# KleistLab/ADAPTed

Hardware: AMD Instinct MI355X
Metric: reads/sec (adapter+polyA detect), RNA004 200k-sample reads (higher is better)
Workload: dtype f32 samples/statistics, f64 cumulative sums + LLR trace

## Files before the change

### adapted_amd/csrc/adapted_hip.hip

```cpp
#include <hip/hip_runtime.h>

#include <cmath>
#include <cstdio>
#include <cstring>
#include <cstdlib>
#include <string>
#include <vector>

#include "adapted_hip.h"
#include "handle.h"
#include "common.h"
__device__ unsigned long long g_dbg[ADP_NDBG] = {0};
__device__ unsigned long long g_bs_tally[ADP_NTALLY][8] = {{0}};
#include "llr_stream.h"
#include "n1_select.h"
#include "n1_fused.h"
#include "peaks.h"
#include "synth.h"
#include "validate.h"
#include "cand_stats2.h"
#include "series_pipe.h"
#include "cnn_topk.h"
#include "cnn_conv.h"
#include "cnn_conv_split.h"
// ... 445 lines not shown
    hipStream_t st = h->stream;
    MbState *mbs = h->mbs.as<MbState>();
    uint32_t *gh = h->ghist.as<uint32_t>(), *gb = h->gbelow.as<uint32_t>();
    unsigned long long *gc = h->gcnt.as<unsigned long long>();
    const int collect = ((long long)minibatch * T >= (1ll << 24)) ? 1 : 0;
    ALLOCCHK(collect && h->cbuf.ensure((size_t)n_mb * N1_CB_CAP * 4));
    uint32_t *cb = h->cbuf.as<uint32_t>();
    int bpm = 4096 / n_mb; if (bpm > 256) bpm = 256; if (bpm < 4) bpm = 4;
    dim3 hg(bpm, n_mb), pg(n_mb);
    const int pdiv = 32;
    int col_div = 1;
    if (T >= 8192) { col_div = T / (pdiv * 96); if (col_div > 64) col_div = 64; if (col_div < 2) col_div = 2; }
    int row_step = (col_div > 1) ? 1 : minibatch / 32; if (row_step < 1) row_step = 1;
    int sb = (minibatch + row_step - 1) / row_step; if (sb > bpm) sb = bpm; if (sb < 1) sb = 1;
    dim3 sg(sb, n_mb);
    const double thr = h->cfg.sig_norm_outlier_thresh;
    const long long fused_min = getenv("ADP_N1_FUSED_MIN") ? atoll(getenv("ADP_N1_FUSED_MIN")) : (1ll << 22);
    if ((long long)minibatch * T >= fused_min && T >= 64) {
        ALLOCCHK(h->cbuf.ensure((size_t)n_mb * N1_CB_CAP * 4) || h->fz.ensure((size_t)n_mb * sizeof(N1Fused)) ||
                 h->fcnt.ensure((size_t)n_mb * 8 * N1F_NCNT) || h->n1heavy.ensure((size_t)n_mb * N1H_WORDS * 4));
        cb = h->cbuf.as<uint32_t>();
        N1Fused *fz = h->fz.as<N1Fused>();
        unsigned long long *fc = h->fcnt.as<unsigned long long>();
        HIPCHK(hipMemsetAsync(fc, 0, (size_t)n_mb * 8 * N1F_NCNT, st));
        uint32_t *hvy = h->n1heavy.as<uint32_t>();
        HIPCHK(hipMemsetAsync(hvy, 0, (size_t)n_mb * N1H_WORDS * 4, st));
        { Scope s(h, !profile ? nullptr : "k_n1 sample passes");
        const int s0 = (col_div > 1 && minibatch >= 64) ? env_int("ADP_N1_S0", 8) : 1;
        for (int mode = 0; mode < 2; mode++) {
            hipLaunchKernelGGL((k_n1_hist<0, SIG>), sg, dim3(N1_THREADS), 0, st, dsig, n, m, T, minibatch, mode, mbs, gh, gb, gc, row_step * (s0 > 1 ? s0 : 1), N1_ALWAYS, cb, 0, col_div, pdiv, tails);
            hipLaunchKernelGGL((k_n1_pick<0, N1_SAMPLE>), pg, dim3(256), 0, st, mbs, gh, gb, gc, mode, thr);
            hipLaunchKernelGGL((k_n1_hist<1, SIG>), sg, dim3(N1_THREADS), 0, st, dsig, n, m, T, minibatch, mode, mbs, gh, gb, gc, row_step, N1_ALWAYS, cb, 0, col_div, pdiv, tails);
            hipLaunchKernelGGL((k_n1_pick<1, N1_SAMPLE>), pg, dim3(256), 0, st, mbs, gh, gb, gc, mode, thr);
            hipLaunchKernelGGL(k_n1_fuse_setup, dim3((n_mb + 63) / 64), dim3(64), 0, st, mbs, fz, n_mb, mode);
        }
        hipLaunchKernelGGL(k_n1_heavy_scan<SIG>, dim3((sb + 3) / 4, n_mb), dim3(N1_THREADS), 0, st, dsig, n, m, T, minibatch, mbs, fz, hvy, row_step * 4, col_div, pdiv, tails);
        hipLaunchKernelGGL(k_n1_heavy_pick, pg, dim3(64), 0, st, mbs, fz, hvy, n_mb); }
        { Scope s(h, !profile ? nullptr : "k_n1_fused");
          hipLaunchKernelGGL(k_n1_fused<SIG>, hg, dim3(N1_THREADS), 0, st, dsig, n, m, T, minibatch, mbs, fz, fc, (float *)cb, hvy, tails); }
        { Scope s(h, !profile ? nullptr : "k_n1_fused_finish");
          hipLaunchKernelGGL(k_n1_fused_finish, pg, dim3(1024), 0, st, mbs, fz, fc, (const float *)cb, thr, (const uint32_t *)hvy); }
    }
    if ((long long)minibatch * T >= fused_min && T >= 64 && bpm < 128) hg = dim3(128, n_mb);
    for (int mode = 0; mode < 2; mode++) {
        hipLaunchKernelGGL((k_n1_hist<0, SIG>), sg, dim3(N1_THREADS), 0, st, dsig, n, m, T, minibatch, mode, mbs, gh, gb, gc, row_step, N1_ALWAYS, cb, 0, col_div, pdiv, tails);
        hipLaunchKernelGGL((k_n1_pick<0, N1_SAMPLE>), pg, dim3(256), 0, st, mbs, gh, gb, gc, mode, thr);
        hipLaunchKernelGGL((k_n1_hist<1, SIG>), sg, dim3(N1_THREADS), 0, st, dsig, n, m, T, minibatch, mode, mbs, gh, gb, gc, row_step, N1_ALWAYS, cb, 0, col_div, pdiv, tails);
        hipLaunchKernelGGL((k_n1_pick<1, N1_SAMPLE>), pg, dim3(256), 0, st, mbs, gh, gb, gc, mode, thr);
        { Scope s(h, !profile ? nullptr : (mode ? "k_n1_hist<1> mad" : "k_n1_hist<1> med"));
          hipLaunchKernelGGL((k_n1_hist<1, SIG>), hg, dim3(N1_THREADS), 0, st, dsig, n, m, T, minibatch, mode, mbs, gh, gb, gc, 1, N1_ALWAYS, cb, collect, 1, 8, tails); }
        hipLaunchKernelGGL((k_n1_pick<1, N1_FULL>), pg, dim3(256), 0, st, mbs, gh, gb, gc, mode, thr);
        hipLaunchKernelGGL(k_n1_finish, pg, dim3(1024), 0, st, mbs, cb, gc, gb, mode, thr);
        hipLaunchKernelGGL((k_n1_hist<0, SIG>), hg, dim3(N1_THREADS), 0, st, dsig, n, m, T, minibatch, mode, mbs, gh, gb, gc, 1, N1_IF_BAD, cb, 0, 1, 8, tails);
        hipLaunchKernelGGL((k_n1_pick<0, N1_FALLBACK>), pg, dim3(256), 0, st, mbs, gh, gb, gc, mode, thr);
        hipLaunchKernelGGL((k_n1_hist<1, SIG>), hg, dim3(N1_THREADS), 0, st, dsig, n, m, T, minibatch, mode, mbs, gh, gb, gc, 1, N1_IF_BAD, cb, 0, 1, 8, tails);
        hipLaunchKernelGGL((k_n1_pick<1, N1_FALLBACK>), pg, dim3(256), 0, st, mbs, gh, gb, gc, mode, thr);
        { Scope s(h, !profile ? nullptr : (mode ? "k_n1_hist<2> mad" : "k_n1_hist<2> med"));
          hipLaunchKernelGGL((k_n1_hist<2, SIG>), hg, dim3(N1_THREADS), 0, st, dsig, n, m, T, minibatch, mode, mbs, gh, gb, gc, 1, N1_IF_NOT_DONE, cb, 0, 1, 8, tails); }
        hipLaunchKernelGGL((k_n1_pick<2, N1_FULL>), pg, dim3(256), 0, st, mbs, gh, gb, gc, mode, thr);
    }
    return 0;
}

struct PhaseSync {
    hipEvent_t wait[3] = {nullptr, nullptr, nullptr};
    hipEvent_t done[3] = {nullptr, nullptr, nullptr};
};

static __device__ __host__ inline SigF32 sig_from(const SigF32 &s, size_t r0, int m) { return SigF32{s.base + r0 * (size_t)m}; }
static __device__ __host__ inline SigI16 sig_from(const SigI16 &s, size_t r0, int m) { return SigI16{s.base + r0 * (size_t)m, s.scale + r0, s.offset + r0, s.full_len + r0}; }
static inline SigIdx sig_subset(const SigF32 &s, const int32_t *sel) { return SigIdx{s.base, sel}; }
static inline SigIdxI16 sig_subset(const SigI16 &s, const int32_t *sel) { return SigIdxI16{s.base, s.scale, s.offset, s.full_len, sel}; }

static void launch_cumsum(adp_handle *h, int n)
{
    const int split = env_int("ADP_CUMSUM_GATHER", 1) != 0;
    hipLaunchKernelGGL(k_cumsum, dim3((n + 63) / 64), dim3(64), 0, h->stream, h->down.as<float>(), h->nvalid.as<int32_t>(), h->Lp, n,
                       h->nck, h->ck.as<double2>(), h->tail.as<double2>(), split);
    if (split)
        hipLaunchKernelGGL(k_cumsum_gather, dim3((n + 63) / 64), dim3(64), 0, h->stream, h->down.as<float>(), h->nvalid.as<int32_t>(), h->Lp, n,
                           h->nck, h->ck.as<double2>(), h->tail.as<double2>());
}

static void launch_polya_peak(adp_handle *h, int n, int mbsize, const double *pkv)
{
    const int grid = n < h->pslots ? n : h->pslots;
    hipLaunchKernelGGL(k_polya_peak, dim3(grid), dim3(64), (size_t)(((h->Lp / 2 + 1) + 8) / 16 + 2) * 4, h->stream, h->trace.as<double>(), h->nvalid.as<int32_t>(), h->Lp,
                       h->bmax.as<double>(), h->bmin.as<double>(), h->nsum, h->adapter_idx.as<int32_t>(), n, mbsize, h->mbs.as<MbState>(),
                       h->pk.as<int32_t>(), h->mk.as<uint32_t>(), h->polya_idx.as<int32_t>(), h->npk.as<int32_t>(), pkv, env_int("ADP_PK_PREFIX", PK_PREFIX));
}

template <class SIG>
static int llr_enqueue(adp_handle *h, SIG dsig, const int32_t *dlen, int n, int m, int minibatch, int flags,
                       adp_row *rows_dev, int rows_kind , int32_t *mb_status_dev, double *mb_params_dev,
                       int upto, const PhaseSync *ps)
{
    int rc = 0;
    const int n_mb = (n + minibatch - 1) / minibatch;
    h->last_n = n; h->last_nmb = n_mb;
    ALLOCCHK(h->mbs.ensure((size_t)n_mb * sizeof(MbState)) || h->ghist.ensure((size_t)n_mb * N1_BINS * 4) || h->gbelow.ensure((size_t)n_mb * 8) || h->gcnt.ensure((size_t)n_mb * 8 * N1_NCNT));
    rc = alloc_all(h, n, true);
    if (rc) return rc;
    hipStream_t st = h->stream;
#ifdef ADP_ABLATE
    sync_ablate(h);
#endif
    if (ps && ps->wait[0]) HIPCHK(hipStreamWaitEvent(st, ps->wait[0], 0));
    MbState *mbs = h->mbs.as<MbState>();
    HIPCHK(hipMemsetAsync(mbs, 0, (size_t)n_mb * sizeof(MbState), st));
    HIPCHK(hipMemsetAsync(h->ghist.p, 0, (size_t)n_mb * N1_BINS * 4, st));
    HIPCHK(hipMemsetAsync(h->gbelow.p, 0, (size_t)n_mb * 8, st));
    HIPCHK(hipMemsetAsync(h->gcnt.p, 0, (size_t)n_mb * 8 * N1_NCNT, st));
    const int T = h->T;
    bool sp_forked = false, sp_done = false;
    if (h->L <= 0) {
        hipLaunchKernelGGL(k_mb_set_status, dim3((n_mb + 255) / 256), dim3(256), 0, st, mbs, n_mb, ADP_MB_EMPTY_TRACE);
        if (ps) for (int k = 0; k < 2; k++) { if (k && ps->wait[k]) HIPCHK(hipStreamWaitEvent(st, ps->wait[k], 0)); if (ps->done[k]) HIPCHK(hipEventRecord(ps->done[k], st)); }
    } else {
        const int32_t *tails = (flags & ADP_TAILS_NAN) ? dlen : nullptr;
        rc = launch_n1(h, dsig, n, m, T, minibatch, n_mb, true, tails);
        if (rc) return rc;
        const bool sp_fused = upto >= 8 && (flags & ADP_WITH_START_PEAK) && h->layout == ADP_LAYOUT_MINIBATCH &&
                              h->cfg.sp_downscale_factor == h->ds && h->off % h->ds == 0 && T > h->off && env_int("ADP_SP_FUSED", 1) != 0;
        if (sp_fused) {
            ALLOCCHK(h->sphead.ensure((size_t)n * sizeof(SpHead)));
            Scope s(h, "k_sp_head");
            hipLaunchKernelGGL(k_sp_head<SIG>, dim3(n), dim3(64), (size_t)64 * h->cfg.sp_downscale_factor * 4, st, dsig, dlen, n, m, h->cfg, h->off, h->sphead.as<SpHead>());
        }
        if (upto >= 2 && sp_fused) {
            { Scope s(h, "k_norm_pool");
              auto kern = (h->ds == 10 && std::is_same<SIG, SigF32>::value && env_int("ADP_NP_PREFETCH", 1)) ? k_norm_pool<SIG, true, 5> : k_norm_pool<SIG, true, 0>;
              hipLaunchKernelGGL(kern, dim3(n), dim3(256), (size_t)NP_TILE * h->ds * 4, st, dsig, m, T, h->off, h->ds, h->L, h->Lp,
                                 minibatch, mbs, h->down.as<float>(), h->nvalid.as<int32_t>(), (const int64_t *)nullptr,
                                 dlen, (flags & ADP_TAILS_NAN) ? 1 : 0, h->sphead.as<SpHead>(), (float)h->cfg.open_pore_pa); }
            const int cov0 = h->off / h->ds, cov1 = cov0 + (T - h->off) / h->ds;
            Scope s(h, "k_sp_tail");
            hipLaunchKernelGGL(k_sp_tail<SIG>, dim3(n), dim3(64), (size_t)64 * h->cfg.sp_downscale_factor * 4, st, dsig, dlen, n, m, h->cfg, cov0, cov1,
                               (const SpHead *)h->sphead.as<SpHead>(), h->sp.as<SpOut>());
            sp_done = true;
        } else if (upto >= 2) {
            Scope s(h, "k_norm_pool");
            const int64_t *rng = nullptr;
            if (h->layout == ADP_LAYOUT_SINGLE_READ) {
                ALLOCCHK(h->rng0.ensure((size_t)n * 16));
                std::vector<int64_t> hr((size_t)2 * n);
                for (int i = 0; i < n; i++) { hr[2 * i] = 0; hr[2 * i + 1] = T; }
                HIPCHK(hipMemcpyAsync(h->rng0.p, hr.data(), (size_t)n * 16, hipMemcpyHostToDevice, st));
                HIPCHK(hipStreamSynchronize(st));
                rng = h->rng0.as<int64_t>();
            }
            auto kern = (h->ds == 10 && !rng && std::is_same<SIG, SigF32>::value && env_int("ADP_NP_PREFETCH", 1)) ? k_norm_pool<SIG, false, 5> : k_norm_pool<SIG, false, 0>;
            hipLaunchKernelGGL(kern, dim3(n), dim3(256), (size_t)NP_TILE * h->ds * 4, st, dsig, m, T, h->off, h->ds, h->L, h->Lp,
                               minibatch, mbs, h->down.as<float>(), h->nvalid.as<int32_t>(), rng,
                               dlen, (flags & ADP_TAILS_NAN) ? 1 : 0, (SpHead *)nullptr, 0.f);
        }
        if (upto >= 2)
            hipLaunchKernelGGL(k_check_empty, dim3((n + 255) / 256), dim3(256), 0, st, h->nvalid.as<int32_t>(), n, minibatch, mbs);
        if (ps && ps->done[0]) HIPCHK(hipEventRecord(ps->done[0], st));
        if (upto >= 8 && (flags & ADP_WITH_START_PEAK) && !sp_fused) {
            HIPCHK(hipEventRecord(h->ev_fork, st));
            HIPCHK(hipStreamWaitEvent(h->stream2, h->ev_fork, 0));
            { Scope s(h, "k_start_peak", h->stream2);
              hipLaunchKernelGGL(k_start_peak<SIG>, dim3(n), dim3(64), (size_t)64 * h->cfg.sp_downscale_factor * 4, h->stream2, dsig, dlen, n, m, h->cfg, h->sp.as<SpOut>()); }
            HIPCHK(hipEventRecord(h->ev_join, h->stream2));
            sp_forked = true;
        }
        if (ps && ps->wait[1]) HIPCHK(hipStreamWaitEvent(st, ps->wait[1], 0));
        if (upto >= 3) {
            Scope s(h, "k_cumsum");
            launch_cumsum(h, n);
        }
        if (upto >= 4) {
            Scope s(h, "k_gains<1>");
            hipLaunchKernelGGL(k_gains<1>, dim3((n + GAINS_WPB - 1) / GAINS_WPB), dim3(64 * GAINS_WPB), 0, st, h->down.as<float>(), h->nvalid.as<int32_t>(), h->Lp, h->nck,
                               h->ck.as<double2>(), h->tail.as<double2>(), h->adapter_idx.as<int32_t>(), minibatch, mbs,
                               h->trace.as<double>(), h->bmax.as<double>(), h->bmin.as<double>(), h->nsum, h->t1.as<int2>(), 0, h->pk.as<int32_t>(), h->npk.as<int32_t>(), h->Lp / 2 + 1, h->gstat.as<double>(), n, h->oh1);
        }
        if (upto >= 5) {
            Scope s(h, "k_adapter_peak");
            hipLaunchKernelGGL(k_adapter_peak, dim3(n), dim3(64), 0, st, h->trace.as<double>(), h->nvalid.as<int32_t>(), h->Lp,
                               h->bmax.as<double>(), h->bmin.as<double>(), h->nsum, h->t1.as<int2>(), minibatch, mbs,
                               h->cfg.adapter_peak_prominence, h->cfg.adapter_peak_rel_height,
                               h->cfg.adapter_peak_width / h->ds, h->adapter_idx.as<int32_t>(), h->gstat.as<double>());
        }
        double *pkvp = (env_int("ADP_PK_VALUES", 1) && h->pkv.cap >= (size_t)n * (h->Lp / 2 + 1) * 8) ? h->pkv.as<double>() : nullptr;
        if (upto >= 6) {
            Scope s(h, "k_gains<2>");
            hipLaunchKernelGGL(k_gains<2>, dim3((n + GAINS_WPB - 1) / GAINS_WPB), dim3(64 * GAINS_WPB), 0, st, h->down.as<float>(), h->nvalid.as<int32_t>(), h->Lp, h->nck,
                               h->ck.as<double2>(), h->tail.as<double2>(), h->adapter_idx.as<int32_t>(), minibatch, mbs,
                               h->trace.as<double>(), h->bmax.as<double>(), h->bmin.as<double>(), h->nsum, h->t1.as<int2>(), 0, h->pk.as<int32_t>(), h->npk.as<int32_t>(), h->Lp / 2 + 1, h->gstat.as<double>(), n, 5, pkvp);
        }
        if (upto >= 7) {
            Scope s(h, "k_polya_peak");
            launch_polya_peak(h, n, minibatch, pkvp);
        }
        if (ps && ps->done[1]) HIPCHK(hipEventRecord(ps->done[1], st));
    }
    if (upto >= 8) {
        if (ps && ps->wait[2]) HIPCHK(hipStreamWaitEvent(st, ps->wait[2], 0));
        if (h->L > 0)
            hipLaunchKernelGGL(k_llr_bounds, dim3((n + 255) / 256), dim3(256), 0, st, h->adapter_idx.as<int32_t>(),
                               h->polya_idx.as<int32_t>(), n, h->ds, h->pos_off, h->bounds.as<int64_t>(), h->topk_none.as<int8_t>(), h->layout == ADP_LAYOUT_SINGLE_READ ? 1 : 0);
        rc = launch_validate(h, dsig, dlen, n, m, 1, minibatch, true);
        if (rc) return rc;
        if (flags & ADP_WITH_START_PEAK) {
            if (sp_forked) HIPCHK(hipStreamWaitEvent(st, h->ev_join, 0));
            else if (!sp_done) {
                Scope s(h, "k_start_peak");
                hipLaunchKernelGGL(k_start_peak<SIG>, dim3(n), dim3(64), (size_t)64 * h->cfg.sp_downscale_factor * 4, st, dsig, dlen, n, m, h->cfg, h->sp.as<SpOut>());
            }
            hipLaunchKernelGGL(k_sp_decorate, dim3((n + 255) / 256), dim3(256), 0, st, h->sp.as<SpOut>(), h->rows.as<adp_row>(), n, 0,
                               (const int32_t *)nullptr);
        }
        if (rows_dev)
            HIPCHK(hipMemcpyAsync(rows_dev, h->rows.p, (size_t)n * sizeof(adp_row), (hipMemcpyKind)rows_kind, st));
    }
    if (mb_status_dev)
        hipLaunchKernelGGL(k_mb_status_out, dim3((n_mb + 255) / 256), dim3(256), 0, st, mbs, n_mb, mb_status_dev);
    if (mb_params_dev)
        hipLaunchKernelGGL(k_mb_params_out, dim3((n_mb + 255) / 256), dim3(256), 0, st, mbs, n_mb, mb_params_dev);
    if (ps && ps->done[2]) HIPCHK(hipEventRecord(ps->done[2], st));
    HIPCHK(hipGetLastError());
    return ADP_OK;
}

static bool trunc_wanted(int flags, const adp_row *rows) { return (flags & ADP_FLAG_TRUNCATED) && rows; }
static int trunc_supported(const adp_handle *h)
{
    const adp_cfg &c = h->cfg;
    const int W = c.median_shift_window;
    if (!c.mvs_detect_check) { g_err = "ADP_FLAG_TRUNCATED needs mvs_detect_check (its tests are the MVS check's)"; return ADP_ERR_UNSUPPORTED; }
    if (c.mvs_detect_overwrite) { g_err = "ADP_FLAG_TRUNCATED does not go with mvs_detect_overwrite"; return ADP_ERR_UNSUPPORTED; }
    if (h->layout == ADP_LAYOUT_SINGLE_READ) { g_err = "ADP_FLAG_TRUNCATED does not go with the single-read layout"; return ADP_ERR_UNSUPPORTED; }
    if (W > PT_WMAX) { g_err = "ADP_FLAG_TRUNCATED: median_shift_window is longer than the tail test holds in LDS (4096)"; return ADP_ERR_UNSUPPORTED; }
    if (c.pA_var_window < 1 || c.pA_mean_window < 1 || c.pA_var_window + 2 >= W || c.pA_mean_window + 2 >= W) {
        g_err = "ADP_FLAG_TRUNCATED: pA_mean_window and pA_var_window must lie in [1, median_shift_window - 3]"; return ADP_ERR_UNSUPPORTED;
    }
    return 0;
}
static int trunc_enqueue_t1(adp_handle *h, const float *dsig, const int32_t *dlen, int n, int m, adp_row *rows)
{
    int8_t *verdict;
    ALLOCCHK(h->pt_sel.ensure((size_t)n * 4));
    RCCHK(sub_carve(h, [&](Carve &c) { verdict = c.take<int8_t>(n); }));
    unsigned int *counts = phase_counts(h, OPW_PT);
    h->pt_looked = true;
    HIPCHK(hipMemsetAsync(counts, 0, 12, h->stream));
    { Scope s(h, "k_pt_t1");
      hipLaunchKernelGGL(k_pt_t1, dim3(n), dim3(64), (size_t)3 * h->cfg.median_shift_window * 4, h->stream, dsig, dlen, n, m, h->cfg, rows, verdict); }
    { Scope s(h, "k_pt_select");
      hipLaunchKernelGGL(k_pt_select, dim3(1), dim3(SEL_THREADS), 0, h->stream, (const int8_t *)verdict, n, h->pt_sel.as<int32_t>(),
                         h->op_used.as<unsigned int>() + 4, counts); }
    return 0;
}
static int trunc_run_t2(adp_handle *h, const float *dsig, const int32_t *dlen, int m, adp_row *rows, int n_t1)
{
    int rc = alloc_all(h, n_t1, false);
    if (rc) return rc;
    const size_t N = (size_t)n_t1;
    int64_t *b2; int32_t *dlen_sub; int8_t *tsub; adp_row *rows2;
    RCCHK(sub_carve(h, [&](Carve &c) {
        b2 = c.take<int64_t>(2 * N); dlen_sub = c.take<int32_t>(N); tsub = c.take<int8_t>(N); rows2 = c.take<adp_row>(N);
    }));
    const int32_t *sel = h->pt_sel.as<int32_t>();
    { Scope s(h, "k_pt_gather");
      hipLaunchKernelGGL(k_pt_gather, dim3((n_t1 + 255) / 256), dim3(256), 0, h->stream, sel, n_t1, m, dlen, (const adp_row *)rows, dlen_sub, b2, tsub); }
    const ValBufs vb{b2, tsub, rows2};
    rc = launch_validate(h, SigIdx{dsig, sel}, dlen_sub, n_t1, m, 1, n_t1, false, &vb, true);
    if (rc) return rc;
    { Scope s(h, "k_pt_merge");
      hipLaunchKernelGGL(k_pt_merge, dim3(n_t1), dim3(64), 0, h->stream, sel, n_t1, (const adp_row *)rows2, rows, phase_counts(h, OPW_PT)); }
    HIPCHK(hipGetLastError());
    return 0;
// ... 780 lines not shown
{
    const int off = h->cfg.min_obs_adapter, ds = h->cfg.downscale_factor;
    const int Lc = (m - off + ds - 1) / ds, L1 = (Lc - 1) / 3 + 1, Lo = 3 * L1 - 2;
    ALLOCCHK(h->cnn_x.ensure((size_t)n_reads * Lc * 4) || h->cnn_sc.ensure((size_t)n_reads * 2 * Lo * 4));
    hipStream_t st = h->stream;
    int rc = alloc_all(h, n_reads, false);
    if (rc) return rc;
    const size_t sp_lds = (size_t)64 * h->cfg.sp_downscale_factor * 4;
    const bool sp_fused = sp_out && cnn_sp_fused(h);
    SpHead *sp_head = nullptr;
    if (sp_fused) {
        ALLOCCHK(h->sphead.ensure((size_t)n_reads * sizeof(SpHead)));
        sp_head = h->sphead.as<SpHead>();
        Scope s(h, "k_sp_head");
        hipLaunchKernelGGL(k_sp_head<SIG>, dim3(n_reads), dim3(64), sp_lds, st, dsig, dlen, n_reads, m, h->cfg, off, sp_head);
    }
    rc = launch_cnn_prepare(h, dsig, n_reads, m, off, ds, Lc, h->cnn_x.as<float>(), sp_head);
    if (rc) return rc;
    if (sp_fused) {
        const int cov0 = off / ds, cov1 = cov0 + (m - off) / ds;
        Scope s(h, "k_sp_tail");
        hipLaunchKernelGGL(k_sp_tail<SIG>, dim3(n_reads), dim3(64), sp_lds, st, dsig, dlen, n_reads, m, h->cfg, cov0, cov1, (const SpHead *)sp_head, sp_out);
    } else if (sp_out) {
        HIPCHK(hipEventRecord(h->ev_fork, st));
        HIPCHK(hipStreamWaitEvent(h->stream2, h->ev_fork, 0));
        { Scope s(h, "k_start_peak", h->stream2);
          hipLaunchKernelGGL(k_start_peak<SIG>, dim3(n_reads), dim3(64), sp_lds, h->stream2, dsig, dlen, n_reads, m, h->cfg, sp_out); }
        HIPCHK(hipEventRecord(h->ev_join, h->stream2));
    }
    struct SpJoin { hipStream_t side; bool armed; ~SpJoin() { if (armed) (void)hipStreamSynchronize(side); } } sp_join{h->stream2, sp_out && !sp_fused};
    rc = cnn_forward_dev(h, h->cnn_x.as<float>(), n_reads, Lc, h->cnn_sc.as<float>());
    if (rc) return rc;
    int kk = 1;
    rc = cnn_predict_dev(h, h->cnn_sc.as<float>(), n_reads, minibatch, Lo, &kk);
    if (rc) return rc;
    if (bounds_dst) HIPCHK(hipMemcpyAsync(bounds_dst, h->bounds.p, (size_t)n_reads * (1 + kk) * 8, (hipMemcpyKind)bounds_kind, st));
    HIPCHK(hipMemsetAsync(h->topk_none.p, 0, (size_t)n_reads, st));
    rc = launch_validate(h, dsig, dlen, n_reads, m, kk, n_reads, false);
    if (rc) return rc;
    if (sp_out) {
        if (!sp_fused) { HIPCHK(hipStreamWaitEvent(st, h->ev_join, 0)); sp_join.armed = false; }
        cnn_sp_decorate(h, sp_out, h->rows.as<adp_row>(), n_reads);
    }
    if (rows_dst) HIPCHK(hipMemcpyAsync(rows_dst, h->rows.p, (size_t)n_reads * sizeof(adp_row), (hipMemcpyKind)rows_kind, st));
    HIPCHK(hipGetLastError());
    return ADP_OK;
}

extern "C++" {
__global__ void k_refine_out(const MbState *mbs, const int32_t *nvalid, const int32_t *polya_idx, const int64_t *ranges, int n,
                             int ds, int64_t *out, int32_t *status)
{
    int r = blockIdx.x * blockDim.x + threadIdx.x;
    if (r >= n) return;
    int st = 0;
    if (mbs[r].status == ADP_MB_MAD_ZERO) st = ADP_F_EXC_MAD_ZERO;
    else if (nvalid[r] <= 0) st = ADP_F_EXC_EMPTY_TRACE;
    int p = polya_idx[r];
    out[r] = (st == 0 && p > 0) ? (int64_t)p * ds + ranges[2 * r] : 0;
    status[r] = st;
}

template <class SIG>
static int refine_chain(adp_handle *h, SIG dsig, const int32_t *dlen, int n, int m, const int64_t *drng, int64_t *dout, int32_t *dstat)
{
    hipStream_t st = h->stream;
    ALLOCCHK(h->mbs.ensure((size_t)n * sizeof(MbState)) || h->ghist.ensure((size_t)n * N1_BINS * 4) || h->gbelow.ensure((size_t)n * 8) || h->gcnt.ensure((size_t)n * 8 * N1_NCNT));
    MbState *mbs = h->mbs.as<MbState>();
    HIPCHK(hipMemsetAsync(mbs, 0, (size_t)n * sizeof(MbState), st));
    HIPCHK(hipMemsetAsync(h->ghist.p, 0, (size_t)n * N1_BINS * 4, st));
    HIPCHK(hipMemsetAsync(h->gbelow.p, 0, (size_t)n * 8, st));
    HIPCHK(hipMemsetAsync(h->adapter_idx.p, 0, (size_t)n * 4, st));
    HIPCHK(hipMemsetAsync(h->gcnt.p, 0, (size_t)n * 8 * N1_NCNT, st));
    { Scope s(h, "k_n1 (refine)");
      int rc = launch_n1(h, dsig, n, m, h->T, 1, n, false);
      if (rc) return rc; }
    { Scope s(h, "k_norm_pool (refine)");
      hipLaunchKernelGGL(k_norm_pool<SIG>, dim3(n), dim3(256), (size_t)NP_TILE * h->ds * 4, st, dsig, m, h->T, h->off, h->ds, h->L, h->Lp, 1, mbs,
                         h->down.as<float>(), h->nvalid.as<int32_t>(), drng, dlen); }
    { Scope s(h, "k_gains (refine)");
      launch_cumsum(h, n);
      hipLaunchKernelGGL(k_gains<1>, dim3((n + GAINS_WPB - 1) / GAINS_WPB), dim3(64 * GAINS_WPB), 0, st, h->down.as<float>(), h->nvalid.as<int32_t>(), h->Lp, h->nck,
                         h->ck.as<double2>(), h->tail.as<double2>(), h->adapter_idx.as<int32_t>(), 1, mbs, h->trace.as<double>(),
                         h->bmax.as<double>(), h->bmin.as<double>(), h->nsum, h->t1.as<int2>(), 1, h->pk.as<int32_t>(), h->npk.as<int32_t>(), h->Lp / 2 + 1, (double *)nullptr, n, 5); }
    { Scope s(h, "k_polya_peak (refine)");
      launch_polya_peak(h, n, 1, nullptr);
      hipLaunchKernelGGL(k_refine_out, dim3((n + 255) / 256), dim3(256), 0, st, mbs, h->nvalid.as<int32_t>(), h->polya_idx.as<int32_t>(),
                         drng, n, h->ds, dout, dstat); }
    return 0;
}
}

static bool cnn_fallback_wanted(const adp_handle *h, int flags, const adp_row *rows)
{
    return (flags & ADP_CNN_FALLBACK) && h->cfg.fallback_to_llr_short_reads && rows;
}
static int cnn_fallback_select(adp_handle *h, const int32_t *dlen, int n, const adp_row *rows, const int64_t *bounds, int bstride)
{
    ALLOCCHK(h->fb_sel.ensure((size_t)n * 4));
    Scope s(h, "k_cnn_fb_select");
    hipLaunchKernelGGL(k_cnn_fb_select, dim3(1), dim3(SEL_THREADS), 0, h->stream, rows, bounds, bstride, dlen, n, 2ll * h->cfg.max_obs_adapter,
                       h->fb_sel.as<int32_t>(), h->op_used.as<unsigned int>() + 2);
    return 0;
}

template <class SIG>
static int cnn_fallback_run(adp_handle *h, SIG dsig, const int32_t *dlen, int m, adp_row *rows, const int64_t *bounds, int bstride, int n_sel)
{
    hipStream_t st = h->stream;
    int rc = alloc_all(h, n_sel, true);
    if (rc) return rc;
    const size_t N = (size_t)n_sel;
    int64_t *drng, *dout, *db2; int32_t *dstat, *dlen_sub; int8_t *topk; adp_row *rows2;
    RCCHK(sub_carve(h, [&](Carve &c) {
        drng = c.take<int64_t>(2 * N); dout = c.take<int64_t>(N); db2 = c.take<int64_t>(2 * N);
        dstat = c.take<int32_t>(N); dlen_sub = c.take<int32_t>(N); topk = c.take<int8_t>(N); rows2 = c.take<adp_row>(N);
    }));
    unsigned int *counts = phase_counts(h, OPW_FB);
    const int32_t *sel = h->fb_sel.as<int32_t>();
    const auto sig = sig_subset(dsig, sel);
    HIPCHK(hipMemsetAsync(counts, 0, 8, st));
    HIPCHK(hipMemsetAsync(topk, 0, N, st));
    { Scope s(h, "k_cnn_fb_gather");
      hipLaunchKernelGGL(k_cnn_fb_gather, dim3((n_sel + 255) / 256), dim3(256), 0, st, sel, n_sel, 0, bounds, bstride, dlen, dlen_sub, drng,
                         (const int64_t *)nullptr, (const int32_t *)nullptr, (int64_t *)nullptr); }
    rc = refine_chain(h, sig, dlen_sub, n_sel, m, drng, dout, dstat);
    if (rc) return rc;
    { Scope s(h, "k_cnn_fb_gather");
      hipLaunchKernelGGL(k_cnn_fb_gather, dim3((n_sel + 255) / 256), dim3(256), 0, st, sel, n_sel, 1, bounds, bstride, dlen, dlen_sub, drng,
                         (const int64_t *)dout, (const int32_t *)dstat, db2); }
    const ValBufs vb{db2, topk, rows2};
    rc = launch_validate(h, sig, dlen_sub, n_sel, m, 1, n_sel, false, &vb);
    if (rc) return rc;
    { Scope s(h, "k_cnn_fb_merge");
      hipLaunchKernelGGL(k_cnn_fb_merge, dim3(n_sel), dim3(64), 0, st, sel, n_sel, (const int64_t *)dout, (const int32_t *)dstat,
                         (const adp_row *)rows2, rows, counts); }
    HIPCHK(hipGetLastError());
    return 0;
}

static bool cnn_second_wanted(int flags, const adp_row *rows) { return (flags & ADP_CNN_SECOND_LLR) && rows; }
static bool cnn_sp_wanted(int flags, const adp_row *rows) { return (flags & ADP_WITH_START_PEAK) && rows; }
static int cnn_second_select(adp_handle *h, int n, const adp_row *rows)
{
    ALLOCCHK(h->so_sel.ensure((size_t)n * 4));
    Scope s(h, "k_cnn_so_select");
    hipLaunchKernelGGL(k_cnn_so_select, dim3(1), dim3(SEL_THREADS), 0, h->stream, rows, n, h->so_sel.as<int32_t>(), h->op_used.as<unsigned int>() + 3);
    return 0;
}

template <class SIG>
static int cnn_second_run(adp_handle *h, SIG dsig, const int32_t *dlen, int n, int m, int minibatch, int flags, adp_row *rows, int n_so)
{
    hipStream_t st = h->stream;
    const int tails = std::is_same<SIG, SigF32>::value ? (flags & ADP_TAILS_NAN) : ADP_TAILS_NAN;
    int rc = llr_enqueue(h, dsig, dlen, n, m, minibatch, tails, nullptr, 0, nullptr, nullptr, 7, nullptr);
    if (rc) return rc;
    const size_t R = (size_t)n, N = (size_t)n_so;
    int64_t *ball, *b2; int32_t *dlen_sub; int8_t *tall, *tsub; adp_row *rows2;
    RCCHK(sub_carve(h, [&](Carve &c) {
        ball = c.take<int64_t>(2 * R); tall = c.take<int8_t>(R);
        b2 = c.take<int64_t>(2 * N); dlen_sub = c.take<int32_t>(N); tsub = c.take<int8_t>(N); rows2 = c.take<adp_row>(N);
    }));
    unsigned int *counts = phase_counts(h, OPW_SO);
    const int32_t *sel = h->so_sel.as<int32_t>();
    const MbState *mbs = h->mbs.as<MbState>();
    HIPCHK(hipMemsetAsync(counts, 0, 12, st));
// ... 441 lines not shown
```

### adapted_amd/csrc/llr_stream.h

```cpp
#pragma once
#include <type_traits>
#include "common.h"
#include "log_cr.h"
#include "wave_stats.h"

#define NP_TILE 512
struct SpHead {
    int32_t valid, max_idx, a2, e0;
    float mx;
    int32_t op_end;
    int32_t op_head, op_body, hit;
    int32_t pad;
};

template <class SIG, bool SP = false, int NQ = 0>
__global__ void __launch_bounds__(256) k_norm_pool(SIG sig, int m, int T, int off, int ds, int L, int Lp,
                                                   int mbsize, const MbState *__restrict__ mbs,
                                                   float *__restrict__ down, int32_t *__restrict__ nvalid,
                                                   const int64_t *__restrict__ ranges, const int32_t *__restrict__ full_len,
                                                   int tails_nan = 0, SpHead *__restrict__ sp_head = nullptr, float sp_thr = 0.f)
{
    extern __shared__ __attribute__((aligned(16))) float tile[];
    __shared__ int s_nan;
    __shared__ __attribute__((aligned(16))) int s_sp[2];
    const int r = blockIdx.x;
    const MbState st = mbs[r / mbsize];
    if (st.status != ADP_MB_OK) { if (threadIdx.x == 0) nvalid[r] = 0; return; }
    const float med = st.med, mad = st.mad, lo = st.lo, hi = st.hi;
    int Lseg = T - off;
    if (ranges) {
        long long a = ranges[2 * r], b = ranges[2 * r + 1];
        long long lim = full_len[r] < T ? full_len[r] : T;
        if (b > lim) b = lim;
        off = (int)a;
        Lseg = (int)(b > a ? b - a : 0);
        L = (Lseg + ds - 1) / ds;
        if (L > Lp) L = Lp;
    }
    const typename SIG::Row row = sig.row(r, m) + off;
    if (threadIdx.x == 0) s_nan = 0;
    int my_nan = 0;
    float sp_mx = 0.f;
    int sp_a2 = 0, sp_e0 = 0, sp_op_end = 0, sp_hit = 0x7fffffff, sp_op = 0x7fffffff;
    const int sp_full = (T - off) / ds;
    const int sp_pb0 = off / ds;
    if (SP) {
        const SpHead hd = sp_head[r];
        sp_mx = hd.mx; sp_a2 = hd.valid ? hd.a2 : 0; sp_e0 = hd.valid ? hd.e0 : 0; sp_op_end = hd.op_end;
        if (threadIdx.x < 2) s_sp[threadIdx.x] = 0x7fffffff;
    }
    int L_ok = L;
    if (tails_nan && !ranges) {
        long long lv = (long long)full_len[r] - off;
        if (lv < Lseg) { if (lv < 0) lv = 0; L_ok = (int)(lv / ds); }
    }
    const int tile_n = NP_TILE * ds;
    const bool vec = row.vec_ok() && ((tile_n & 3) == 0);
    const bool fast_div = fdiv_ok(mad);
    const float rmad = 1.0f / mad;
    auto norm1 = [&](float c) {
        c = c < lo ? lo : c;
        c = c > hi ? hi : c;
        return fast_div ? fdiv_shared(c - med, mad, rmad) : (c - med) / mad;
    };
    const bool use_pf = NQ > 0 && vec && tile_n / 4 == NQ * 256;
    float4 pre[NQ > 0 ? NQ : 1];
    auto fetch = [&](int tb_) {
        const int base_ = tb_ * ds;
        const typename SIG::Row rowb = row + base_;
#pragma unroll
        for (int u = 0; u < (NQ > 0 ? NQ : 1); u++) {
            const int q = threadIdx.x + u * 256;
            const int idx = base_ + 4 * q;
            float4 v = make_float4(0.f, 0.f, 0.f, 0.f);
            if (idx + 3 < Lseg) v = rowb.f4s(q);
            else {
                if (idx < Lseg) v.x = row[idx];
                if (idx + 1 < Lseg) v.y = row[idx + 1];
                if (idx + 2 < Lseg) v.z = row[idx + 2];
            }
            pre[u] = v;
        }
    };
    if (use_pf && L_ok > 0 && L > 0) fetch(0);
    for (int tb = 0; tb < L; tb += NP_TILE) {
        const int base = tb * ds;
        if (tb >= L_ok) {
// ... 190 lines not shown
        for (int l2 = 0; l2 < LPG; l2 += PFL) {
#pragma unroll
            for (int d = 0; d < PFL; d++) {
                const int line = g0 * LPG + l2 + d, j1 = line * 2 * CK, slot = 2 * (l2 + d);
                if (j1 < n) block(j1, slot, q[d][0]);
                if (j1 + CK < n) block(j1 + CK, slot + 1, q[d][1]);
                ldl(line + PFL, q[d]);
            }
        }
        ws_sync();
        const int q0 = g0 * CSUM_Q;
#pragma unroll
        for (int it = 0; it < 8; it++) {
            const int rd = 8 * it + (ln >> 3), pc = ln & 7;
            const int nrd = __shfl(n, rd);
            if (r0 + rd < n_reads && (q0 + pc) * CK < nrd) {
                const csum_d2 v = cks[rd * (CSUM_Q + 1) + pc];
                ck[(size_t)(r0 + rd) * nck + q0 + pc] = make_double2(v.x, v.y);
            }
        }
        ws_sync();
    }
    if (r < n_reads) tail[r] = t;
}

static __device__ __forceinline__ double recip_refined(double b)
{
    const double y0 = __builtin_amdgcn_rcp(b);
    const double e0 = __builtin_fma(-b, y0, 1.0);
    const double y1 = __builtin_fma(y0, e0, y0);
    const double e1 = __builtin_fma(-b, y1, 1.0);
    return __builtin_fma(y1, e1, y1);
}
static __device__ __forceinline__ double div_by_len(double a, double b, double y)
{
    const double q0 = a * y;
    const double r = __builtin_fma(-b, q0, a);
    return __builtin_fma(r, y, q0);
}

static __device__ __noinline__ double gains_log_slow(double u) { return log(u); }
static __device__ __forceinline__ double var_seg(double c2hi, double c2lo, double chi, double clo, double dl)
{
    const double y = recip_refined(dl);
    double mu = div_by_len(chi - clo, dl, y);
    return div_by_len(c2hi - c2lo, dl, y) - mu * mu;
}

static __device__ __forceinline__ double wave_shr1_f64(double x, double fill)
{
    int2 v = __builtin_bit_cast(int2, x), f = __builtin_bit_cast(int2, fill);
    v.x = __builtin_amdgcn_update_dpp(f.x, v.x, 0x138 , 0xf, 0xf, false);
    v.y = __builtin_amdgcn_update_dpp(f.y, v.y, 0x138, 0xf, 0xf, false);
    return __builtin_bit_cast(double, v);
}
static __device__ __forceinline__ double readlane_f64(double x, int lane)
{
    int2 v = __builtin_bit_cast(int2, x);
    v.x = __builtin_amdgcn_readlane(v.x, lane);
    v.y = __builtin_amdgcn_readlane(v.y, lane);
    return __builtin_bit_cast(double, v);
}

#ifndef GAINS_UNROLL
#define GAINS_UNROLL 1
#endif
#ifndef GAINS_SU
#define GAINS_SU 4
#endif
#ifndef GAINS_EU
#define GAINS_EU 4
#endif
#ifndef GAINS_WPB
#define GAINS_WPB 4
#endif
template <int PASS>
__global__ void __launch_bounds__(64 * GAINS_WPB, 4) k_gains(const float *__restrict__ down, const int32_t *__restrict__ nvalid, int Lp, int nck,
                                              const double2 *__restrict__ ck, const double2 *__restrict__ tail,
                                              const int32_t *__restrict__ adapter_idx, int mbsize,
                                              const MbState *__restrict__ mbs, double *__restrict__ trace,
                                              double *__restrict__ bmax, double *__restrict__ bmin, int nsum,
                                              int2 *__restrict__ t1, int sanitize, int32_t *__restrict__ pk_all,
                                              int32_t *__restrict__ npk_all, int pk_stride, double *__restrict__ gstat, int n_reads, int oh1,
                                              double *__restrict__ pkv_all = nullptr)
{
    __shared__ __attribute__((aligned(16))) double sg_[GAINS_WPB][64 * (CK + 1)];
    __shared__ __attribute__((aligned(16))) double lt_[3 * LOGCR_N];
    LDS double *sg = (LDS double *)sg_[threadIdx.x >> 6];
    const int r = blockIdx.x * GAINS_WPB + (threadIdx.x >> 6);
    const int ln = lane_id();
    for (int i = threadIdx.x; i < 3 * LOGCR_N; i += 64 * GAINS_WPB) lt_[i] = g_logcr_table[i];
    __syncthreads();
    if (r >= n_reads) return;
    const LDS double *lt = (const LDS double *)lt_;
    auto flog = [&](double v) { return log_cr_impl(v, lt, [](double u) { return gains_log_slow(u); }); };
    if (mbs[r / mbsize].status != ADP_MB_OK) return;
    const int n = nvalid[r];
    if (n <= 0) return;
    int start = 0, oh = oh1, ot = 5;
    if (PASS == 2) {
        start = adapter_idx[r];
        if (start < 0) return;
        oh = 1; ot = 1;
    }
    const int E = n - 1;
    const float *s = down + (size_t)r * Lp;
    const double2 *c = ck + (size_t)r * nck;
    double *g = trace + (size_t)r * Lp;
    const double2 te = tail[r];
    double cs = 0.0, c2s = 0.0;
    if (PASS == 2 && start > 0) {
        int q = start / CK;
        double2 p = c[q];
        double a = p.x, b = p.y;
        for (int j = q * CK; j < start; j++) { double v = (double)s[j]; a += v; b += v * v; }
        cs = a; c2s = b;
    }
    double vs;
    {
        double v = (start == E) ? 0.0 : var_seg(te.y, c2s, te.x, cs, (double)(E - start));
        vs = (double)(E - start) * flog(v);
    }
    int first_pos = 0x7fffffff, last_pos = -1;
    double st_s1 = 0.0, st_s2 = 0.0;
    int st_nan = 0;
    const bool emit = (PASS == 2 || sanitize) && pk_all;
    int32_t *pk = emit ? pk_all + (size_t)r * pk_stride : nullptr;
    double *pkv = (emit && pkv_all) ? pkv_all + (size_t)r * pk_stride : nullptr;
    int npk = 0;
    bool plateau = false;
    double carry1 = 0.0, carry2 = 0.0;
    for (int tb = 0; tb < n; tb += TRACE_TILE) {
        ws_sync();
        const int i0 = tb + ln * CK;
        const float4 *s4 = reinterpret_cast<const float4 *>(s + (i0 < Lp ? i0 : 0));
        double a = 0.0, b = 0.0;
        if (i0 < n) { double2 p = c[i0 / CK]; a = p.x; b = p.y; }
        double mx = -__builtin_inf(), mn = __builtin_inf();
        double dlh = (double)(i0 - start), dlt = (double)(E - i0);
        auto point = [&](auto interior_c, int t, int i, float qf) {
            constexpr bool INTERIOR = decltype(interior_c)::value;
            double gi = 0.0;
            const double lh_len = dlh, lt_len = dlt;
            dlh += 1.0; dlt -= 1.0;
            if (INTERIOR || i < n) {
                if (INTERIOR || (i >= start + oh && i < E - ot)) {
                    double vh = var_seg(b, c2s, a, cs, lh_len);
                    double vt = var_seg(te.y, b, te.x, a, lt_len);
#ifdef ADP_GAINS_LOG_CR
                    double lh = log_cr_fast(vh, lt), ll = log_cr_fast(vt, lt);
#else
                    double lh = log_1ulp_fast(vh, lt), ll = log_1ulp_fast(vt, lt);
#endif
                    if (!(log_cr_ok(vh) && log_cr_ok(vt))) {
                        if (!log_cr_ok(vh)) lh = gains_log_slow(vh);
                        if (!log_cr_ok(vt)) ll = gains_log_slow(vt);
                    }
                    double h = lh_len * lh;
                    double tl = lt_len * ll;
                    gi = vs - (h + tl);
                }
                if (PASS == 1 && !(gi <= 0.0)) { first_pos = min(first_pos, i); last_pos = i; }
                const bool finite = __builtin_fabs(gi) < __builtin_inf();
                if (PASS == 1) { if (gi == gi) { st_s1 += gi; st_s2 += gi * gi; } else st_nan++; }
                if (PASS == 1 && !sanitize) {
                    if (finite) { mx = gi > mx ? gi : mx; mn = gi < mn ? gi : mn; }
                    else {
                        double m1 = (gi != gi) ? __builtin_inf() : gi;
                        mx = m1 > mx ? m1 : mx;
                        if (gi == gi) mn = gi < mn ? gi : mn;
                    }
                } else {
                    double x = gi;
                    if (!finite) x = (x != x) ? 0.0 : (x > 0 ? 1.7976931348623157e308 : -1.7976931348623157e308);
                    mx = x > mx ? x : mx;
                    mn = x < mn ? x : mn;
                }
                double v = (double)qf;
                a += v;
                b += v * v;
            }
            sg[ln * (CK + 1) + t] = gi;
        };
        const bool interior = tb >= start + oh && tb + TRACE_TILE <= E - ot;
        if (interior) {
#pragma unroll GAINS_UNROLL
            for (int tq = 0; tq < CK / 4; tq++) {
                const float4 q4 = s4[tq];
                const float qv[4] = {q4.x, q4.y, q4.z, q4.w};
#pragma unroll
                for (int u = 0; u < 4; u++) point(std::true_type{}, tq * 4 + u, i0 + tq * 4 + u, qv[u]);
            }
        } else {
#pragma unroll GAINS_UNROLL
            for (int tq = 0; tq < CK / 4; tq++) {
                const float4 q4 = s4[tq];
                const float qv[4] = {q4.x, q4.y, q4.z, q4.w};
#pragma unroll
                for (int u = 0; u < 4; u++) point(std::false_type{}, tq * 4 + u, i0 + tq * 4 + u, qv[u]);
            }
        }
        {
            double w;
            w = __shfl_xor(mx, 1); mx = w > mx ? w : mx;
            w = __shfl_xor(mx, 2); mx = w > mx ? w : mx;
            w = __shfl_xor(mn, 1); mn = w < mn ? w : mn;
            w = __shfl_xor(mn, 2); mn = w < mn ? w : mn;
            int blk = tb / SUMBLK + (ln >> 2);
            if ((ln & 3) == 0 && blk < nsum && (tb + (ln >> 2) * SUMBLK) < n) {
                bmax[(size_t)r * nsum + blk] = mx;
                bmin[(size_t)r * nsum + blk] = mn;
            }
        }
        ws_sync();
        auto sanit = [](double x) {
            if (x != x) x = 0.0;
            else if (__builtin_isinf(x)) x = x > 0 ? 1.7976931348623157e308 : -1.7976931348623157e308;
            return x;
        };
        auto sval = [&](int e) { return sanit(sg[(e / CK) * (CK + 1) + (e % CK)]); };
        if (!emit) {
#pragma unroll GAINS_SU
            for (int k = 0; k < CK; k++) {
                int e = k * 64 + ln;
                int i = tb + e;
                if (i < n) g[i] = sg[(e / CK) * (CK + 1) + (e % CK)];
            }
        } else {
            double p1 = carry1, p2 = carry2;
#pragma unroll GAINS_EU
            for (int k = 0; k < CK; k++) {
                const int e = k * 64 + ln;
                const int i = tb + e;
                const int j = i - 1;
                const double raw = sg[(e / CK) * (CK + 1) + (e % CK)];
                if (i < n) g[i] = raw;
                const double xn = sanit(raw);
                const double xj = wave_shr1_f64(xn, p1);
                const double xp = wave_shr1_f64(xj, p2);
                p1 = readlane_f64(xn, 63); p2 = readlane_f64(xn, 62);
                bool pkf = false;
                if (i < n && j >= 1) {
                    if (xp < xj) {
                        if (xn < xj) pkf = true;
                        else if (xn == xj && !(xj == 0.0 && j >= E - ot)) plateau = true;
                    }
                }
                unsigned long long mk = __ballot(pkf);
                if (pkf) { const int at = npk + __popcll(mk & ((1ull << ln) - 1ull)); pk[at] = j; if (pkv) pkv[at] = xj; }
                npk += __popcll(mk);
            }
            const int last = min(TRACE_TILE, n - tb) - 1;
            double c1 = sval(last), c2v = (last >= 1) ? sval(last - 1) : carry1;
            carry2 = c2v; carry1 = c1;
        }
    }
    if (emit) {
        plateau = __any(plateau);
        if (ln == 0) npk_all[r] = plateau ? -1 : npk;
    }
    if (PASS == 1) {
        first_pos = wave_min(first_pos);
        last_pos = wave_max(last_pos);
        if (ln == 0) {
            int st = (last_pos < 0) ? 0 : first_pos;
            int en = (last_pos < 0) ? n - 1 : last_pos;
            t1[r] = make_int2(st, en);
        }
        st_s1 = wave_sum(st_s1); st_s2 = wave_sum(st_s2); st_nan = wave_sum(st_nan);
        if (ln == 0 && gstat) { gstat[3 * r] = st_s1; gstat[3 * r + 1] = st_s2; gstat[3 * r + 2] = (double)st_nan; }
    }
}
```

### adapted_amd/csrc/log_cr.h

```cpp
#pragma once
#include <stdint.h>
#include <string.h>

#include "log_cr_table.h"

#if defined(__HIPCC__)
#define LOGCR_FN static __device__ __forceinline__
#define LOGCR_FMA(a, b, c) __builtin_fma(a, b, c)
__device__ const double g_logcr_table[3 * LOGCR_N] = LOGCR_TABLE;
#else
#include <math.h>
#define LOGCR_FN static inline
#define LOGCR_FMA(a, b, c) fma(a, b, c)
#endif

LOGCR_FN bool log_cr_ok(double x)
{
    uint64_t ix;
    memcpy(&ix, &x, 8);
    return ix - 0x0010000000000000ULL < 0x7FF0000000000000ULL - 0x0010000000000000ULL;
}

template <class TabPtr>
LOGCR_FN double log_cr_fast(double x, TabPtr tab)
{
    uint64_t ix;
    memcpy(&ix, &x, 8);
    const uint64_t tmp = ix - LOGCR_OFF;
    const int i = (int)((tmp >> 45) & 127u);
    const int32_t k = (int32_t)(uint32_t)(tmp >> 32) >> 20;
    const uint64_t iz = ix - (tmp & 0xFFF0000000000000ULL);
    double z;
    memcpy(&z, &iz, 8);
    const double invc = tab[3 * i], lch = tab[3 * i + 1], lcl = tab[3 * i + 2];
    const double r = LOGCR_FMA(z, invc, -1.0);
    const double kd = (double)k;
    const double a = kd * LOGCR_LN2HI;
    const double t1 = a + lch;
    const double e1 = lch - (t1 - a);
    const double t2 = t1 + r;
    const double bb = t2 - t1;
    const double e2 = (t1 - (t2 - bb)) + (r - bb);
    const double rr = r * r;
    const double rrl = LOGCR_FMA(r, r, -rr);
    const double h = -0.5 * rr;
    const double t3 = t2 + h;
    const double e3 = h - (t3 - t2);
    double q = LOGCR_Q7;
    q = LOGCR_FMA(q, r, LOGCR_Q6);
    q = LOGCR_FMA(q, r, LOGCR_Q5);
    q = LOGCR_FMA(q, r, LOGCR_Q4);
    q = LOGCR_FMA(q, r, LOGCR_Q3);
    q = LOGCR_FMA(q, r, LOGCR_Q2);
    q = LOGCR_FMA(q, r, LOGCR_Q1);
    q = LOGCR_FMA(q, r, LOGCR_Q0);
    double lo = LOGCR_FMA(kd, LOGCR_LN2LO, lcl);
    lo += e1;
    lo += e2;
    lo += e3;
    lo = LOGCR_FMA(-0.5, rrl, lo);
    lo = LOGCR_FMA(r * rr, q, lo);
    return t3 + lo;
}

template <class TabPtr>
LOGCR_FN double log_1ulp_fast(double x, TabPtr tab)
{
    uint64_t ix;
    memcpy(&ix, &x, 8);
    const uint64_t tmp = ix - LOGCR_OFF;
    const int i = (int)((tmp >> 45) & 127u);
    const int32_t k = (int32_t)(uint32_t)(tmp >> 32) >> 20;
    const uint64_t iz = ix - (tmp & 0xFFF0000000000000ULL);
    double z;
    memcpy(&z, &iz, 8);
    const double invc = tab[3 * i], lch = tab[3 * i + 1], lcl = tab[3 * i + 2];
    const double r = LOGCR_FMA(z, invc, -1.0);
    const double kd = (double)k;
    const double hi = LOGCR_FMA(kd, LOGCR_LN2HI, lch);
    double lo = LOGCR_FMA(kd, LOGCR_LN2LO, lcl);
    double q = LOGCR_Q6;
    q = LOGCR_FMA(q, r, LOGCR_Q5);
    q = LOGCR_FMA(q, r, LOGCR_Q4);
    q = LOGCR_FMA(q, r, LOGCR_Q3);
    q = LOGCR_FMA(q, r, LOGCR_Q2);
    q = LOGCR_FMA(q, r, LOGCR_Q1);
    q = LOGCR_FMA(q, r, LOGCR_Q0);
    const double rr = r * r;
    lo = LOGCR_FMA(r * rr, q, lo);
    lo = LOGCR_FMA(-0.5, rr, lo);
    const double sum = hi + r;
    const double err = r - (sum - hi);
    return sum + (err + lo);
}

template <class TabPtr, class Fallback>
LOGCR_FN double log_cr_impl(double x, TabPtr tab, Fallback fallback)
{
    if (!log_cr_ok(x)) return fallback(x);
    return log_cr_fast(x, tab);
}

#if !defined(__HIPCC__)
static const double logcr_host_table[3 * LOGCR_N] = LOGCR_TABLE;
static inline double log_cr_host(double x)
{
    return log_cr_impl(x, logcr_host_table, [](double v) { return log(v); });
}
static inline double log_1ulp_host(double x) { return log_cr_ok(x) ? log_1ulp_fast(x, logcr_host_table) : log(x); }
#endif
```

Measured before the change: 1.060 million.

## Add speculative fast path for interior gains tiles with fallback redo

```diff
diff --git a/adapted_amd/csrc/adapted_hip.hip b/adapted_amd/csrc/adapted_hip.hip
--- a/adapted_amd/csrc/adapted_hip.hip
+++ b/adapted_amd/csrc/adapted_hip.hip
@@ -551,6 +551,8 @@
                            h->nck, h->ck.as<double2>(), h->tail.as<double2>());
 }
 
+static int gains_tile_fast() { return env_int("ADP_GAINS_TILE_FAST", 1) != 0; }
+
 static void launch_polya_peak(adp_handle *h, int n, int mbsize, const double *pkv)
 {
     const int grid = n < h->pslots ? n : h->pslots;
@@ -643,7 +645,7 @@
             Scope s(h, "k_gains<1>");
             hipLaunchKernelGGL(k_gains<1>, dim3((n + GAINS_WPB - 1) / GAINS_WPB), dim3(64 * GAINS_WPB), 0, st, h->down.as<float>(), h->nvalid.as<int32_t>(), h->Lp, h->nck,
                                h->ck.as<double2>(), h->tail.as<double2>(), h->adapter_idx.as<int32_t>(), minibatch, mbs,
-                               h->trace.as<double>(), h->bmax.as<double>(), h->bmin.as<double>(), h->nsum, h->t1.as<int2>(), 0, h->pk.as<int32_t>(), h->npk.as<int32_t>(), h->Lp / 2 + 1, h->gstat.as<double>(), n, h->oh1);
+                               h->trace.as<double>(), h->bmax.as<double>(), h->bmin.as<double>(), h->nsum, h->t1.as<int2>(), 0, h->pk.as<int32_t>(), h->npk.as<int32_t>(), h->Lp / 2 + 1, h->gstat.as<double>(), n, h->oh1, nullptr, gains_tile_fast());
         }
         if (upto >= 5) {
             Scope s(h, "k_adapter_peak");
@@ -657,7 +659,7 @@
             Scope s(h, "k_gains<2>");
             hipLaunchKernelGGL(k_gains<2>, dim3((n + GAINS_WPB - 1) / GAINS_WPB), dim3(64 * GAINS_WPB), 0, st, h->down.as<float>(), h->nvalid.as<int32_t>(), h->Lp, h->nck,
                                h->ck.as<double2>(), h->tail.as<double2>(), h->adapter_idx.as<int32_t>(), minibatch, mbs,
-                               h->trace.as<double>(), h->bmax.as<double>(), h->bmin.as<double>(), h->nsum, h->t1.as<int2>(), 0, h->pk.as<int32_t>(), h->npk.as<int32_t>(), h->Lp / 2 + 1, h->gstat.as<double>(), n, 5, pkvp);
+                               h->trace.as<double>(), h->bmax.as<double>(), h->bmin.as<double>(), h->nsum, h->t1.as<int2>(), 0, h->pk.as<int32_t>(), h->npk.as<int32_t>(), h->Lp / 2 + 1, h->gstat.as<double>(), n, 5, pkvp, gains_tile_fast());
         }
         if (upto >= 7) {
             Scope s(h, "k_polya_peak");
@@ -1604,7 +1606,7 @@
       launch_cumsum(h, n);
       hipLaunchKernelGGL(k_gains<1>, dim3((n + GAINS_WPB - 1) / GAINS_WPB), dim3(64 * GAINS_WPB), 0, st, h->down.as<float>(), h->nvalid.as<int32_t>(), h->Lp, h->nck,
                          h->ck.as<double2>(), h->tail.as<double2>(), h->adapter_idx.as<int32_t>(), 1, mbs, h->trace.as<double>(),
-                         h->bmax.as<double>(), h->bmin.as<double>(), h->nsum, h->t1.as<int2>(), 1, h->pk.as<int32_t>(), h->npk.as<int32_t>(), h->Lp / 2 + 1, (double *)nullptr, n, 5); }
+                         h->bmax.as<double>(), h->bmin.as<double>(), h->nsum, h->t1.as<int2>(), 1, h->pk.as<int32_t>(), h->npk.as<int32_t>(), h->Lp / 2 + 1, (double *)nullptr, n, 5, nullptr, gains_tile_fast()); }
     { Scope s(h, "k_polya_peak (refine)");
       launch_polya_peak(h, n, 1, nullptr);
       hipLaunchKernelGGL(k_refine_out, dim3((n + 255) / 256), dim3(256), 0, st, mbs, h->nvalid.as<int32_t>(), h->polya_idx.as<int32_t>(),
diff --git a/adapted_amd/csrc/llr_stream.h b/adapted_amd/csrc/llr_stream.h
--- a/adapted_amd/csrc/llr_stream.h
+++ b/adapted_amd/csrc/llr_stream.h
@@ -3,6 +3,8 @@
 #include "common.h"
 #include "log_cr.h"
 #include "wave_stats.h"
+
+extern __device__ unsigned long long g_dbg[ADP_NDBG];
 
 #define NP_TILE 512
 struct SpHead {
@@ -359,7 +361,7 @@
                                               double *__restrict__ bmax, double *__restrict__ bmin, int nsum,
                                               int2 *__restrict__ t1, int sanitize, int32_t *__restrict__ pk_all,
                                               int32_t *__restrict__ npk_all, int pk_stride, double *__restrict__ gstat, int n_reads, int oh1,
-                                              double *__restrict__ pkv_all = nullptr)
+                                              double *__restrict__ pkv_all = nullptr, int tile_fast = 0)
 {
     __shared__ __attribute__((aligned(16))) double sg_[GAINS_WPB][64 * (CK + 1)];
     __shared__ __attribute__((aligned(16))) double lt_[3 * LOGCR_N];
@@ -398,6 +400,8 @@
         double v = (start == E) ? 0.0 : var_seg(te.y, c2s, te.x, cs, (double)(E - start));
         vs = (double)(E - start) * flog(v);
     }
+    const bool fast_read = tile_fast && __all(__builtin_fabs(vs) < __builtin_inf() && __builtin_bit_cast(uint64_t, vs) != 0x8000000000000000ULL);
+    int n_fast = 0, n_redo = 0;
     int first_pos = 0x7fffffff, last_pos = -1;
     double st_s1 = 0.0, st_s2 = 0.0;
     int st_nan = 0;
@@ -460,7 +464,60 @@
             sg[ln * (CK + 1) + t] = gi;
         };
         const bool interior = tb >= start + oh && tb + TRACE_TILE <= E - ot;
-        if (interior) {
+        bool committed = false;
+        if (__builtin_amdgcn_readfirstlane((int)(interior && fast_read))) {
+            uint32_t fh = 0u, ft = 0u;
+            int f_first = first_pos, f_last = last_pos;
+            double f_s2 = st_s2;
+            if (PASS == 1) sg[ln * (CK + 1) + CK] = st_s1;
+#pragma unroll GAINS_UNROLL
+            for (int tq = 0; tq < CK / 4; tq++) {
+                const float4 q4 = s4[tq];
+                const float qv[4] = {q4.x, q4.y, q4.z, q4.w};
+#pragma unroll
+                for (int u = 0; u < 4; u++) {
+                    const int t = tq * 4 + u, i = i0 + t;
+                    const double lh_len = dlh, lt_len = dlt;
+                    dlh += 1.0; dlt -= 1.0;
+                    const double vh = var_seg(b, c2s, a, cs, lh_len);
+                    const double vt = var_seg(te.y, b, te.x, a, lt_len);
+                    fh = max(fh, (uint32_t)(__builtin_bit_cast(uint64_t, vh) >> 32) - 0x00100000u);
+                    ft = max(ft, (uint32_t)(__builtin_bit_cast(uint64_t, vt) >> 32) - 0x00100000u);
+#ifdef ADP_GAINS_LOG_CR
+                    const double lh = log_cr_fast(vh, lt), ll = log_cr_fast(vt, lt);
+#else
+                    const double lh = log_1ulp_fast(vh, lt), ll = log_1ulp_fast(vt, lt);
+#endif
+                    const double h = lh_len * lh;
+                    const double tl = lt_len * ll;
+                    const double gi = vs - (h + tl);
+                    if (PASS == 1) {
+                        if (!(gi <= 0.0)) { f_first = min(f_first, i); f_last = i; }
+                        st_s1 += gi; f_s2 += gi * gi;
+                    }
+                    mx = __builtin_fmax(gi, mx);
+                    mn = __builtin_fmin(gi, mn);
+                    const double v = (double)qv[u];
+                    a += v;
+                    b += v * v;
+                    sg[ln * (CK + 1) + t] = gi;
+                }
+            }
+            committed = !__any(max(fh, ft) >= 0x7FE00000u);
+            if (committed) {
+                n_fast++;
+                if (PASS == 1) { first_pos = f_first; last_pos = f_last; st_s2 = f_s2; }
+            } else {
+                n_redo++;
+                if (PASS == 1) st_s1 = sg[ln * (CK + 1) + CK];
+                const double2 p = c[i0 / CK];
+                a = p.x; b = p.y;
+                mx = -__builtin_inf(); mn = __builtin_inf();
+                dlh = (double)(i0 - start); dlt = (double)(E - i0);
+            }
+        }
+        if (committed) {
+        } else if (interior) {
 #pragma unroll GAINS_UNROLL
             for (int tq = 0; tq < CK / 4; tq++) {
                 const float4 q4 = s4[tq];
@@ -497,12 +554,41 @@
         };
         auto sval = [&](int e) { return sanit(sg[(e / CK) * (CK + 1) + (e % CK)]); };
         if (!emit) {
+            if (committed) {
 #pragma unroll GAINS_SU
+                for (int k = 0; k < CK; k++) {
+                    const int e = k * 64 + ln;
+                    g[tb + e] = sg[(e / CK) * (CK + 1) + (e % CK)];
+                }
+            } else {
+#pragma unroll GAINS_SU
+                for (int k = 0; k < CK; k++) {
+                    int e = k * 64 + ln;
+                    int i = tb + e;
+                    if (i < n) g[i] = sg[(e / CK) * (CK + 1) + (e % CK)];
+                }
+            }
+        } else if (committed) {
+            double p1 = carry1, p2 = carry2;
+#pragma unroll GAINS_EU
             for (int k = 0; k < CK; k++) {
-                int e = k * 64 + ln;
-                int i = tb + e;
-                if (i < n) g[i] = sg[(e / CK) * (CK + 1) + (e % CK)];
-            }
+                const int e = k * 64 + ln;
+                const int j = tb + e - 1;
+                const double xn = sg[(e / CK) * (CK + 1) + (e % CK)];
+                g[tb + e] = xn;
+                const double xj = wave_shr1_f64(xn, p1);
+                const double xp = wave_shr1_f64(xj, p2);
+                p1 = readlane_f64(xn, 63); p2 = readlane_f64(xn, 62);
+                bool pkf = false;
+                if (xp < xj) {
+                    if (xn < xj) pkf = true;
+                    else if (xn == xj) plateau = true;
+                }
+                unsigned long long mk = __ballot(pkf);
+                if (pkf) { const int at = npk + __popcll(mk & ((1ull << ln) - 1ull)); pk[at] = j; if (pkv) pkv[at] = xj; }
+                npk += __popcll(mk);
+            }
+            carry1 = sg[63 * (CK + 1) + CK - 1]; carry2 = sg[63 * (CK + 1) + CK - 2];
         } else {
             double p1 = carry1, p2 = carry2;
 #pragma unroll GAINS_EU
@@ -536,6 +622,8 @@
         plateau = __any(plateau);
         if (ln == 0) npk_all[r] = plateau ? -1 : npk;
     }
+    if (ln == 0 && n_fast) atomicAdd(&g_dbg[76], (unsigned long long)n_fast);
+    if (ln == 0 && n_redo) atomicAdd(&g_dbg[77], (unsigned long long)n_redo);
     if (PASS == 1) {
         first_pos = wave_min(first_pos);
         last_pos = wave_max(last_pos);
diff --git a/adapted_amd/csrc/log_cr.h b/adapted_amd/csrc/log_cr.h
--- a/adapted_amd/csrc/log_cr.h
+++ b/adapted_amd/csrc/log_cr.h
@@ -21,6 +21,14 @@
     return ix - 0x0010000000000000ULL < 0x7FF0000000000000ULL - 0x0010000000000000ULL;
 }
 
+LOGCR_FN double logcr_kd(int32_t k)
+{
+    const uint64_t ib = 0x4330000000000000ULL | (uint64_t)((uint32_t)k ^ 0x80000000u);
+    double d;
+    memcpy(&d, &ib, 8);
+    return d - 4503601774854144.0;
+}
+
 template <class TabPtr>
 LOGCR_FN double log_cr_fast(double x, TabPtr tab)
 {
@@ -34,7 +42,7 @@
     memcpy(&z, &iz, 8);
     const double invc = tab[3 * i], lch = tab[3 * i + 1], lcl = tab[3 * i + 2];
     const double r = LOGCR_FMA(z, invc, -1.0);
-    const double kd = (double)k;
+    const double kd = logcr_kd(k);
     const double a = kd * LOGCR_LN2HI;
     const double t1 = a + lch;
     const double e1 = lch - (t1 - a);
@@ -76,7 +84,7 @@
     memcpy(&z, &iz, 8);
     const double invc = tab[3 * i], lch = tab[3 * i + 1], lcl = tab[3 * i + 2];
     const double r = LOGCR_FMA(z, invc, -1.0);
-    const double kd = (double)k;
+    const double kd = logcr_kd(k);
     const double hi = LOGCR_FMA(kd, LOGCR_LN2HI, lch);
     double lo = LOGCR_FMA(kd, LOGCR_LN2LO, lcl);
     double q = LOGCR_Q6;
@@ -108,4 +116,5 @@
     return log_cr_impl(x, logcr_host_table, [](double v) { return log(v); });
 }
 static inline double log_1ulp_host(double x) { return log_cr_ok(x) ? log_1ulp_fast(x, logcr_host_table) : log(x); }
+static inline double logcr_kd_host(int32_t k) { return logcr_kd(k); }
 #endif
```

After: 1.080 million (median of 6 runs). 1.9% higher.
